# 0xk0ry/HTR-VT

Hardware: AMD Instinct MI355X
Metric: line-images/sec (64x1024, global B=128, 128 per GPU) fwd+bwd+CTC (higher is better)
Workload: dtype bf16; 1 GPU; HTR-VT (d768/4L/6h, nb_cls 80) training step: fwd + fused CTC + bwd + AdamW; image=1x64x1024, batch_per_gpu=128, global_batch=128, mask=span 0.4/8 (run/iam.sh), parallelism=dp1, graph_replay=False

## Files before the change

htr-vt_amd/_lib.py:

```python
from __future__ import annotations

import ctypes as C
import os

import torch

_HERE = os.path.dirname(os.path.abspath(__file__))
LIB_PATH = os.environ.get("HTRVT_LIB") or os.path.join(_HERE, "lib", "libhtrvt_hip.so")

F32, BF16 = 0, 1
KMAJOR, MNMAJOR = 0, 1
GATHER_NONE, GATHER_CONV_FWD, GATHER_CONV_DGRAD, GATHER_CONV_WGRAD = 0, 1, 2, 3

vp, i32, i64, f32, f64 = C.c_void_p, C.c_int32, C.c_int64, C.c_float, C.c_double


class RelayoutJob(C.Structure):
    _fields_ = [
        ("src", vp), ("dst0", vp), ("dst1", vp), ("kind", i32), ("d0", i32), ("d1", i32),
        ("taps", i32), ("cpad_in", i32), ("cpad_out", i32), ("row_taps", i32), ("tap0", i32),
        ("tile0", i32), ("tiles_x", i32), ("reserved_", i32 * 2),
    ]


# ... 6 lines not shown
        ("dtype", i32), ("a_layout", i32), ("b_layout", i32), ("gather", i32),
        ("M", i32), ("N", i32), ("K", i32),
        ("lda", i64), ("ldb", i64), ("ldc", i64),
        ("batch", i32), ("batch_inner", i32),
        ("sA_o", i64), ("sA_i", i64), ("sB_o", i64), ("sB_i", i64), ("sC_o", i64), ("sC_i", i64),
        ("split_k", i32), ("splitk_ws", vp),
        ("nB", i32), ("Hi", i32), ("Wi", i32), ("Ci", i32), ("Ho", i32), ("Wo", i32), ("Co", i32),
        ("kh", i32), ("kw", i32), ("sh", i32), ("sw", i32), ("ph", i32), ("pw", i32), ("Cpad", i32),
        ("cls_h", i32), ("cls_w", i32),
        ("A2", vp),
        ("alpha", f32), ("act", i32), ("c_f32", i32), ("accumulate", i32), ("tile", i32),
        ("bias", vp), ("colscale", vp), ("preact", vp), ("residual", vp), ("colstats", vp),
        ("relu_src", vp), ("bnb_x", vp * 2), ("bnb_mean", vp * 2), ("bnb_rstd", vp * 2), ("bnb_partial", vp * 2),
        ("bnb_tile0", i32), ("relu_scale", vp), ("relu_shift", vp), ("relu_bits", i32),
        ("A", vp), ("B", vp), ("C", vp),
    ]


PROTOTYPES = {
    "htrvt_version": (i32, []),
    "htrvt_last_error": (C.c_char_p, []),
    "htrvt_last_kernel": (C.c_char_p, []),
    "htrvt_gemm": (i32, [C.POINTER(GemmDesc), vp]),
    "htrvt_gemm_num_mtiles": (i32, [C.POINTER(GemmDesc)]),
    "htrvt_gemm_wgrad_tiling": (i32, [C.POINTER(GemmDesc), C.POINTER(i32), C.POINTER(i32)]),
    "htrvt_gemm_dgrad_merged_tiles": (i32, [C.POINTER(GemmDesc)]),
    "htrvt_img_stats": (i32, [vp, vp, i32, i32, f32, i32, vp]),
    "htrvt_conv1_fwd": (i32, [vp, vp, vp, vp, vp, i32, i32, i32, i32, i32, i32, vp]),
    "htrvt_stem_stats_rows": (i32, [i32, i32]),
    "htrvt_stem_stats": (i32, [vp, vp, vp, vp, vp, i32, i32, i32, i32, i32, vp]),
# ... 8 lines not shown
    "htrvt_softmax_rows": (i32, [vp, vp, i64, i32, i32, vp, i64, vp]),
    "htrvt_attn_supported": (i32, [i32, i32, i32]),
    "htrvt_attn_fwd": (i32, [vp, vp, vp, vp, i32, i32, i32, i32, f32, i32, vp]),
    "htrvt_attn_bwd": (i32, [vp, vp, vp, vp, vp, vp, vp, vp, i32, i32, i32, i32, f32, i32, vp]),
    "htrvt_seq_whiten_fwd": (i32, [vp, vp, vp, i32, i32, f32, i32, vp]),
    "htrvt_seq_whiten_bwd": (i32, [vp, vp, vp, vp, i32, i32, i32, i32, i32, vp]),
    "htrvt_layernorm_bwd_blocks": (i32, [i64]),
    "htrvt_layernorm_bwd": (i32, [vp, vp, vp, vp, vp, vp, vp, vp, i64, i32, i32, vp]),
    "htrvt_softmax_bwd_rows": (i32, [vp, vp, vp, i64, i32, f32, i32, vp]),
    "htrvt_colsum_workspace_floats": (C.c_size_t, [i64, i32]),
    "htrvt_colsum": (i32, [vp, i64, i32, i64, vp, vp, i32, i32, vp, vp]),
    "htrvt_rowsum_f32": (i32, [vp, i32, i32, vp, vp]),
    "htrvt_bn_bwd_blocks": (i32, [i64]),
    "htrvt_bn_bwd_reduce": (i32, [vp, vp, vp, vp, vp, vp, i64, i32, i32, vp]),
    "htrvt_bn_bwd_finalize": (i32, [vp, i32, i32, f32, vp, vp, vp, vp, vp, vp, vp]),
    "htrvt_bn_bwd_apply": (i32, [vp, vp, vp, vp, vp, vp, i64, i32, i32, vp]),
    "htrvt_bn_bwd_apply2": (i32, [vp, vp, vp, vp, vp, vp, vp, i64, i32, i32, vp]),
    "htrvt_maxpool_bwd": (i32, [vp, vp, vp, vp, vp, vp, i32, i32, i32, i32, i32, vp]),
    "htrvt_pool_tokens_bwd": (i32, [vp, vp, vp, vp, i32, i32, i32, i32, i32, vp]),
    "htrvt_conv1_bwd_rows": (i32, [i32, i32]),
    "htrvt_conv1_bwd_row_floats": (i32, [i32]),
    "htrvt_conv1_bwd": (i32, [vp] * 12 + [i32, i32, i32, i32, i32, i32, vp]),
    "htrvt_conv1_wgrad_blocks": (i32, [i32, i32]),
    "htrvt_conv1_wgrad": (i32, [vp, vp, vp, vp, vp, i32, i32, i32, i32, i32, i32, vp]),
    "htrvt_pack_conv_weight": (i32, [vp, vp, vp, i32, i32, i32, i32, i32, i32, vp]),
    "htrvt_pack_conv_weight_slots": (i32, [vp, vp, vp, i32, i32, i32, i32, i32, i32, i32, i32, vp]),
    "htrvt_unpack_conv_wgrad": (i32, [vp, vp, i32, i32, i32, i32, vp]),
    "htrvt_cast_f32": (i32, [vp, vp, i64, i32, vp]),
    "htrvt_relayout_plan": (i32, [vp, i32]),
    "htrvt_relayout": (i32, [vp, i32, i32, i32, vp]),
# ... 78 lines not shown
```

htr-vt_amd/csrc/bwd.hip:

```cpp
#include "common.h"

using namespace htrvt;

namespace {

constexpr int NT = 256;
constexpr int MAXC = 4;

inline int grid_for(long long work_items, int cap = 256 * 8) {
  long long g = (work_items + NT - 1) / NT;
  if (g > cap) g = cap;
  if (g < 1) g = 1;
  return (int)g;
}

template <typename T>
__global__ __launch_bounds__(NT) void seq_whiten_bwd_kernel(const float* __restrict__ dy, const float* __restrict__ y,
                                                            const float* __restrict__ stats, T* __restrict__ dx, int NC,
                                                            int C, int ldo) {
  __shared__ float red[8];
  const float* dys = dy + (long long)blockIdx.x * NC;
  const float* ys = y + (long long)blockIdx.x * NC;
  float s1 = 0.f, s2 = 0.f;
  for (int i = threadIdx.x; i < NC; i += NT) {
// ... 798 lines not shown
  dim3 grid(htrvt_bn_bwd_blocks(npix));
  DISPATCH_T(dtype, hipLaunchKernelGGL(bn_bwd_reduce_kernel<T>, grid, dim3(NT), smem, (hipStream_t)stream, (const T*)dy,
                                       (const T*)yact, (const T*)x, mean, rstd, partial, (long long)npix, C, nthr));
  return check_launch("bn_bwd_reduce");
}

extern "C" int htrvt_bn_bwd_finalize(const float* partial, int rows, int C, float count, const float* gamma,
                                     const float* mean, const float* rstd, float* dgamma, float* dbeta, float* coef,
                                     void* stream) {
  HTRVT_REQUIRE(partial && gamma && mean && rstd && dgamma && dbeta && coef, "htrvt_bn_bwd_finalize: null argument");
  hipLaunchKernelGGL(bn_bwd_finalize_kernel, dim3((C + 63) / 64), dim3(64), 0, (hipStream_t)stream, partial, rows, C, count,
                     gamma, mean, rstd, dgamma, dbeta, coef);
  return check_launch("bn_bwd_finalize");
}

extern "C" int htrvt_bn_bwd_apply(const void* dy, const void* yact, const void* x, const float* coef, void* dx, void* gout,
                                  int64_t npix, int C, int dtype, void* stream) {
  const int ch = dtype == HTRVT_BF16 ? 8 : 4;
  HTRVT_REQUIRE(C % ch == 0, "htrvt_bn_bwd_apply: C=%d unsupported", C);
  const long long nvec = npix * (C / ch);
  dim3 grid(grid_for(nvec));
  if (nvec * 16 >= BN_STREAM_BYTES) {
    DISPATCH_T(dtype, hipLaunchKernelGGL((bn_bwd_apply_kernel<T, true>), grid, dim3(NT), (size_t)3 * C * sizeof(float), (hipStream_t)stream, (const T*)dy,
                                         (const T*)yact, (const T*)x, coef, (T*)dx, (T*)gout, nvec, C));
  } else {
    DISPATCH_T(dtype, hipLaunchKernelGGL((bn_bwd_apply_kernel<T, false>), grid, dim3(NT), (size_t)3 * C * sizeof(float), (hipStream_t)stream, (const T*)dy,
                                         (const T*)yact, (const T*)x, coef, (T*)dx, (T*)gout, nvec, C));
  }
  return check_launch("bn_bwd_apply");
}
// ... 111 lines not shown
```

htr-vt_amd/csrc/gemm.hip:

```cpp
#include "gemm_common.h"

using namespace htrvt;

namespace {

constexpr int NTHREADS = 256;

template <typename T, int ROWS, int LAYOUT>
struct TileGeom {
  static constexpr int SZ = ET<T>::SZ;
  static constexpr int BK = ET<T>::BK;
  static constexpr int STRIDE = (LAYOUT == HTRVT_KMAJOR) ? 128 : (ROWS * SZ + 64);
  static constexpr int LROWS = (LAYOUT == HTRVT_KMAJOR) ? ROWS : BK;
  static constexpr int BYTES = STRIDE * LROWS;
  static constexpr int NLOAD = ROWS / 32;
  static constexpr int CPR = (LAYOUT == HTRVT_KMAJOR) ? 8 : (ROWS * SZ / 16);
};

template <typename T, int ROWS, int LAYOUT, int ROLE>
struct Loader {
  using G = TileGeom<T, ROWS, LAYOUT>;
  static constexpr int SZ = G::SZ, CH = ET<T>::CH, NL = G::NLOAD;
  uint4 reg[NL];
  const char* ptr[NL];
// ... 246 lines not shown
            for (int j = 0; j < TN; ++j)
              acc[i][j] = __builtin_amdgcn_mfma_f32_32x32x2f32((&fa[i].x)[jj], (&fb[j].x)[jj], acc[i][j], 0, 0, 0);
      }
    }
    if (more) {
      la.commit(nxt);
      lb.commit(nxt + GA::BYTES);
    }
    __syncthreads();
  }

  gemm_epilogue<T, TM, TN, 2, BN, NTHREADS>(acc, p, Cb, coff, m0 + wm * TM * 32, n0 + wn * TN * 32, wm, n0, tile_m, lane, smem);
}

__global__ __launch_bounds__(NTHREADS) void splitk_reduce_kernel(const float* __restrict__ ws, float* __restrict__ C, int M, int N,
                                                                 long long ldc, int nsl, int accumulate) {
  const long long mn = (long long)M * N;
  const int n4 = N >> 2;
  for (long long i = (long long)blockIdx.x * NTHREADS + threadIdx.x; i < (long long)M * n4; i += (long long)gridDim.x * NTHREADS) {
    const int m = (int)(i / n4), c = (int)(i - (long long)m * n4);
    const float4* src = reinterpret_cast<const float4*>(ws + (long long)m * N) + c;
    float4 a = *src;
    int z = 1;
    for (; z + 8 <= nsl; z += 8) {
      float4 b[8];
#pragma unroll
      for (int u = 0; u < 8; ++u) b[u] = *reinterpret_cast<const float4*>(reinterpret_cast<const float*>(src) + (z + u) * mn);
#pragma unroll
      for (int u = 0; u < 8; ++u) {
        a.x += b[u].x; a.y += b[u].y; a.z += b[u].z; a.w += b[u].w;
      }
// ... 203 lines not shown
      HTRVT_REQUIRE(diff > 0 && diff + (long long)d->nB * d->Ho * d->Wo * d->Co * 2 < (1ll << 31) - 64,
                    "htrvt_gemm: A2 must lie behind A, both inside 2 GiB");
      p.tapsel[p.ntapsel++] = (unsigned char)(d->kh * d->kw);
      p.extra_off = (unsigned)diff;
    }
    HTRVT_REQUIRE(d->M == d->nB * p.Hq * p.Wq && d->K == p.ntapsel * d->Cpad && d->N == d->Ci,
                  "htrvt_gemm: parity-class dgrad extents inconsistent (expected M=%d K=%d)", d->nB * p.Hq * p.Wq,
                  p.ntapsel * d->Cpad);
  }
  p.tappack = 0;
  for (int t = 0; t < 12; ++t) p.tappack |= (unsigned long long)(p.tapsel[t] & 15) << (4 * t);
  const int zdim = p.split_k > 1 ? p.split_k : (d->batch > 1 ? d->batch : 1);
  HTRVT_REQUIRE((long long)p.tiles_m * p.tiles_n < (1ll << 31) && zdim < 65536, "htrvt_gemm: grid too large");
  hipStream_t st = (hipStream_t)stream;
  p.slab_stride = 0;
  if (p.split_k > 1 && d->splitk_ws != nullptr) {
    p.C = reinterpret_cast<char*>(d->splitk_ws);
    p.ldc = d->N;
    p.accumulate = 0;
    p.slab_stride = (long long)d->M * d->N;
    const int rc = launch_main(d, p, bm, bn, zdim, st);
    if (rc) return rc;
    long long items = (long long)d->M * (d->N / 4);
    int grid = (int)((items + NTHREADS - 1) / NTHREADS);
    if (grid > 2048) grid = 2048;
    hipLaunchKernelGGL(splitk_reduce_kernel, dim3(grid), dim3(NTHREADS), 0, st, d->splitk_ws, reinterpret_cast<float*>(d->C), d->M,
                       d->N, (long long)d->ldc, p.split_k, d->accumulate);
    return check_launch("splitk_reduce");
  }
  return launch_main(d, p, bm, bn, zdim, st);
}

static int launch_main(const HtrvtGemmDesc* d, KParams& p, int bm, int bn, int zdim, hipStream_t st) {
  const bool cls = d->gather == HTRVT_GATHER_CONV_DGRAD && d->cls_h >= 0;
  const bool fused_bwd = d->relu_src != nullptr || d->bnb_partial[0] != nullptr;
  if (d->dtype == HTRVT_BF16 && d->tile != 1) {
    KParams q = p;
    int r = gemm8p_try_launch(d, q, zdim, st);
    if (r != 0) return r < 0 ? r : 0;
    q = p;
    r = gemm8pt_try_launch(d, q, zdim, st);
    if (r != 0) return r < 0 ? r : 0;
// ... 21 lines not shown
```

htr-vt_amd/csrc/gemm8p.hip:

```cpp
#include <stdlib.h>

#include "gemm_common.h"

using namespace htrvt;

namespace htrvt {
int gemm8p_dispatch_plain(int bn, int epi, const KParams&, int, hipStream_t);
int gemm8pp_dispatch_plain(int bn, int epi, const KParams&, int nwg, hipStream_t);
int gemm8pt_dispatch(const KParams&, int zdim, hipStream_t);
int gemm8p_dispatch_conv(int bn, int gather, int epi, const KParams&, int, hipStream_t);
}

namespace {

int ilog2_exact(int v) {
  if (v <= 0 || (v & (v - 1))) return -1;
  int s = 0;
  while ((1 << s) < v) ++s;
  return s;
}

bool extents_ok(const HtrvtGemmDesc* d) {
  const long long lim = (1ll << 31) - 64;
  long long a, b = (long long)d->N * d->ldb * 2;
// ... 48 lines not shown
}

bool gemm8pt_serves(const HtrvtGemmDesc* d) {
  if (d->tile != 0 && d->tile != 16) return false;
  if (d->dtype != HTRVT_BF16 || d->gather != HTRVT_GATHER_NONE || d->a_layout != HTRVT_MNMAJOR || d->b_layout != HTRVT_MNMAJOR) return false;
  if (!d->c_f32 || d->batch > 1 || d->M < 256 || d->N < 256 || d->K < 256) return false;
  if (d->tile == 0 && (long long)((d->M + 255) / 256) * ((d->N + 255) / 256) < 16) return false;
  if ((d->M & 7) || (d->N & 7) || (d->lda & 7) || (d->ldb & 7) || (d->ldc & 3)) return false;
  if ((reinterpret_cast<unsigned long long>(d->A) & 15) || (reinterpret_cast<unsigned long long>(d->B) & 15) || (reinterpret_cast<unsigned long long>(d->C) & 15)) return false;
  if (d->bias != nullptr || d->act != 0 || d->preact != nullptr || d->residual != nullptr || d->colstats != nullptr || d->colscale != nullptr) return false;
  const long long lim = (1ll << 31) - 64;
  if ((long long)d->K * d->lda * 2 >= lim || (long long)d->K * d->ldb * 2 >= lim) return false;
  return true;
}

int gemm8pt_try_launch(const HtrvtGemmDesc* d, KParams& p, int zdim, hipStream_t st) {
  if (!gemm8pt_serves(d)) return 0;
  if (p.split_k > 1 ? p.slab_stride == 0 : p.accumulate != 0) return 0;
  p.tiles_m = (d->M + 255) / 256;
  p.tiles_n = (d->N + 255) / 256;
  return gemm8pt_dispatch(p, zdim, st);
}

int gemm8p_try_launch(const HtrvtGemmDesc* d, KParams& p, int zdim, hipStream_t st) {
  if (!gemm8p_serves(d)) return 0;
  const int bn = gemm8p_pick_bn(d);
  int epi = 0;
  if (d->residual != nullptr) epi |= E_RES;
  if (d->act == 1) epi |= E_GELU;
  if (d->act == 2) epi |= E_GELUGRAD;
// ... 42 lines not shown
```

htr-vt_amd/csrc/gemm8p_impl.h:

```cpp
#pragma once
#include <type_traits>

#include "gemm_common.h"

using namespace htrvt;

namespace g8 {

constexpr int BK = 64;

typedef int i32x2_t __attribute__((ext_vector_type(2)));
typedef float f32x4_t __attribute__((ext_vector_type(4)));
using I0 = std::integral_constant<int, 0>;
using I1 = std::integral_constant<int, 1>;

template <int BN_, int WARPS_M_, int WARPS_N_>
struct Cfg {
  static constexpr int BM = 256, BN = BN_, WARPS_M = WARPS_M_, WARPS_N = WARPS_N_;
  static_assert(WARPS_M * WARPS_N == 8, "8 waves");
  static constexpr int HM = BM / 2, HN = BN / 2;
  static constexpr int SM = HM / WARPS_M, SN = HN / WARPS_N;
  static constexpr int MT = SM / 16, NT = SN / 16;
  static_assert(SM % 16 == 0 && SN % 16 == 0 && (NT == 2 || NT == 3), "quadrant shape");
  static constexpr int A_HALF = HM * 128, B_HALF = HN * 128;
// ... 259 lines not shown
  if ((wave >> 2) == 1) __builtin_amdgcn_s_barrier();
}

template <class F>
__device__ __forceinline__ void mfma_phase(F&& mma) {
  __builtin_amdgcn_s_barrier();
  asm volatile("s_waitcnt lgkmcnt(0)" ::: "memory");
  __builtin_amdgcn_sched_barrier(0);
  __builtin_amdgcn_s_setprio(1);
  mma();
  __builtin_amdgcn_s_setprio(0);
  __builtin_amdgcn_sched_barrier(0);
  __builtin_amdgcn_s_barrier();
}

template <int BUFI, int LGKM1, class RA, class RB, class SA, class SB, class MMA>
__device__ __forceinline__ void ktile8p(RA& readA, RB& readB, SA& stageA, SB& stageB, MMA& mma) {
  using BX = std::integral_constant<int, BUFI>;
  using BY = std::integral_constant<int, BUFI ^ 1>;
  readB(I0{}, BX{});
  __builtin_amdgcn_sched_barrier(0);
  readA(I0{}, BX{});
  __builtin_amdgcn_sched_barrier(0);
  stageA(I1{}, BY{});
  asm volatile("s_waitcnt lgkmcnt(%0)" ::"n"(LGKM1) : "memory");
  mfma_phase([&] { mma(I0{}, I0{}); });
  readB(I1{}, BX{});
  __builtin_amdgcn_sched_barrier(0);
  stageB(I0{}, BX{});
  mfma_phase([&] { mma(I0{}, I1{}); });
  readA(I1{}, BX{});
  __builtin_amdgcn_sched_barrier(0);
  stageA(I0{}, BX{});
  mfma_phase([&] { mma(I1{}, I1{}); });
  stageB(I1{}, BX{});
  asm volatile("s_waitcnt vmcnt(6)" ::: "memory");
  mfma_phase([&] { mma(I1{}, I0{}); });
}

__device__ __forceinline__ void drain8p(int wave) {
  if ((wave >> 2) == 0) __builtin_amdgcn_s_barrier();
  asm volatile("s_waitcnt vmcnt(0)" ::: "memory");
}

template <class C, int GATHER, int EPI, class P>
__device__ __forceinline__ void gemm8p_body(const P& p, const int block_x) {
  constexpr int MT = C::MT, NT = C::NT;
  extern __shared__ __attribute__((aligned(16))) char smem[];

  const int id = xcd_tile_id(block_x, p.tiles_m * p.tiles_n);
// ... 340 lines not shown
```

htr-vt_amd/csrc/gemm8pt_impl.h:

```cpp
#pragma once
#include "gemm8p_impl.h"

namespace g8 {

__device__ __forceinline__ int tswz(int k) { return ((k & 3) | (((k >> 3) & 1) << 2)) << 1; }

struct TLoad {
  unsigned off[2][2];
  int klocal[2];
  unsigned kstep;
  int k0;
  i32x4_t rsrc;

  __device__ __forceinline__ void init(const char* base, long long ld, int mn0, int dim, int kbeg, int wave, int lane) {
    rsrc = make_rsrc(base);
    k0 = kbeg;
    kstep = (unsigned)(BK * ld * 2);
#pragma unroll
    for (int i = 0; i < 2; ++i) {
      const int pi = wave + 8 * i;
      const int kl = 4 * pi + (lane >> 4);
      klocal[i] = kl;
      const int cs = (lane & 15) ^ tswz(kl);
#pragma unroll
// ... 8 lines not shown
#pragma unroll
    for (int i = 0; i < 2; ++i) {
      const unsigned voff = (k0 + klocal[i] < kend) ? off[H][i] : OOB;
      dma16(rsrc, __builtin_amdgcn_readfirstlane(lds_half + (wave + 8 * i) * 1024), voff);
    }
    if constexpr (H == 1) {
      k0 += BK;
#pragma unroll
      for (int i = 0; i < 2; ++i)
#pragma unroll
        for (int h = 0; h < 2; ++h) off[h][i] = off[h][i] < OOB ? off[h][i] + kstep : OOB;
    }
  }
};

template <class P>
__device__ __forceinline__ void gemm8pt_body(const P& p, const int block_x) {
  using C = Cfg<256, 2, 4>;
  constexpr int MT = C::MT, NT = C::NT;
  extern __shared__ __attribute__((aligned(16))) char smem[];

  const int id = xcd_tile_id(block_x, p.tiles_m * p.tiles_n);
  const int tile_m = id / p.tiles_n, tile_n = id - tile_m * p.tiles_n;
  const int m0 = tile_m * C::BM, n0 = tile_n * C::BN;
  const int z = blockIdx.z;
  const int kbeg = z * p.kchunk;
  const int kend = (kbeg + p.kchunk < p.K) ? kbeg + p.kchunk : p.K;

  const int lane = threadIdx.x & 63;
  const int wave = __builtin_amdgcn_readfirstlane(threadIdx.x >> 6);
  const int wr = wave / C::WARPS_N, wc = wave - wr * C::WARPS_N;
// ... 53 lines not shown
  };
  auto readB = [&](auto yc, auto bufc) {
    constexpr int Y = decltype(yc)::value;
    const char* half = smem + decltype(bufc)::value * C::BUF + (Y ? OB1 : OB0);
#pragma unroll
    for (int j = 0; j < NT; ++j) {
      fb[Y][j][0] = ldtr(half, rdB[j]);
      fb[Y][j][1] = ldtr(half, rdB[j] + 32 * 256);
    }
  };
  auto mma = [&](auto xc, auto yc) {
    constexpr int X = decltype(xc)::value, Y = decltype(yc)::value;
    mma_quadrant<false>(acc[X][Y], fb[Y], fa);
  };
  constexpr int LGKM1 = 15;
  prologue8p(stageA, stageB, wave);
  int kt = 0;
  for (; kt + 1 < nkt; kt += 2) {
    ktile8p<0, LGKM1>(readA, readB, stageA, stageB, mma);
    ktile8p<1, LGKM1>(readA, readB, stageA, stageB, mma);
  }
  if (kt < nkt) ktile8p<0, LGKM1>(readA, readB, stageA, stageB, mma);
  drain8p(wave);

  const int g = lane >> 4, jr = lane & 15;
  float* Cf = reinterpret_cast<float*>(p.C) + (p.slab_stride > 0 ? (long long)z * p.slab_stride : 0ll);
  const float alpha = p.alpha;
#pragma unroll
  for (int x = 0; x < 2; ++x)
#pragma unroll
    for (int i = 0; i < MT; ++i) {
      const int m = m0 + x * C::HM + wr * C::SM + 16 * i + jr;
      if (m < p.M) {
        float* row = Cf + (long long)m * p.ldc;
#pragma unroll
        for (int y = 0; y < 2; ++y)
#pragma unroll
          for (int j = 0; j < NT; ++j) {
            const int n = n0 + y * C::HN + wc * C::SN + 16 * j + 4 * g;
            if (n < p.N) *reinterpret_cast<f32x4_t*>(row + n) = acc[x][y][i][j] * alpha;
          }
      }
    }
}

__global__ __launch_bounds__(512) void gemm8pt_kernel(const KParams p) {
  typedef const __attribute__((address_space(4))) KParams KP;
  (void)p;
  KP* kp = (KP*)__builtin_amdgcn_kernarg_segment_ptr();
  gemm8pt_body(*kp, (int)blockIdx.x);
}

inline int launch_t(const KParams& p, int zdim, hipStream_t st) {
  using C = Cfg<256, 2, 4>;
  if (int rc = allow_dynamic_lds<gemm8pt_kernel>(C::LDS_BYTES, "gemm8pt_kernel")) return rc;
  hipLaunchKernelGGL(gemm8pt_kernel, dim3(p.tiles_m * p.tiles_n, 1, zdim), dim3(512), C::LDS_BYTES, st, p);
  set_last_kernel("gemm8pt_kernel");
  const int rc = check_launch("gemm8pt_kernel");
  return rc ? rc : 1;
}

}
```

htr-vt_amd/csrc/gemm_common.h:

```cpp
#pragma once
#include "common.h"

namespace htrvt {

typedef __attribute__((ext_vector_type(8))) __bf16 bf16x8_t;
typedef __attribute__((ext_vector_type(4))) short s16x4_t;
typedef __attribute__((ext_vector_type(8))) short s16x8_t;
typedef __attribute__((ext_vector_type(16))) float f32x16_t;
typedef int i32x4_t __attribute__((ext_vector_type(4)));

constexpr unsigned OOB = 0x80000000u;

__device__ __forceinline__ void dma16(const i32x4_t& rsrc, unsigned lds_addr, unsigned voff) {
  unsigned keep;
  asm volatile(
      "s_nop 4\n\t"
      "s_mov_b32 %0, m0\n\t"
      "s_mov_b32 m0, %2\n\t"
      "s_nop 0\n\t"
      "buffer_load_dwordx4 %1, %3, 0 offen lds\n\t"
      "s_mov_b32 m0, %0"
      : "=&s"(keep)
      : "v"(voff), "s"(lds_addr), "s"(rsrc)
      : "memory");
// ... 51 lines not shown
  int wo_shift, howo_shift;
  int cls_h, cls_w, Hq, Wq, ntapsel;
  int wq_shift, hwq_shift;
  unsigned char tapsel[12];
  unsigned long long tappack;
  unsigned extra_off;
  const char* relu_src;
  int relu_bits;
  const char* bnb_x[2];
  const float* bnb_mean[2];
  const float* bnb_rstd[2];
  float* bnb_partial[2];
  int bnb_tile0;
  const float* relu_sc;
  const float* relu_sf;
};

inline bool gemm_small_m_prefers_bn128(const HtrvtGemmDesc* d) {
  if (d->tile != 0 || d->gather != HTRVT_GATHER_NONE || d->dtype != HTRVT_BF16) return false;
  if (d->a_layout != HTRVT_KMAJOR || d->b_layout != HTRVT_KMAJOR || d->batch > 1 || d->split_k > 1) return false;
  if (d->N > 1024 || d->N % 128 != 0) return false;
  const long long tiles192 = (long long)((d->M + 255) / 256) * ((d->N + 191) / 192);
  return tiles192 <= 128;
}

__device__ __forceinline__ float gelu_erf(float x) { return 0.5f * x * (1.0f + erff(x * 0.70710678118654752440f)); }
__device__ __forceinline__ float gelu_erf_grad(float x) {
  return 0.5f * (1.0f + erff(x * 0.70710678118654752440f)) + x * 0.39894228040143267794f * __expf(-0.5f * x * x);
}

// ... 129 lines not shown
          q += red[(w * BN + c) * 2 + 1];
        }
        float* dst = p.colstats + (long long)tile_m * 2 * p.N;
        dst[n] = a;
        dst[p.N + n] = q;
      }
    }
  }
}

int gemm_dma_try_launch(const HtrvtGemmDesc* d, KParams& p, int zdim, hipStream_t st);
int gemm_dma_num_mtiles(const HtrvtGemmDesc* d);
int gemm8p_try_launch(const HtrvtGemmDesc* d, KParams& p, int zdim, hipStream_t st);
int gemm8pt_try_launch(const HtrvtGemmDesc* d, KParams& p, int zdim, hipStream_t st);
bool gemm8pt_serves(const HtrvtGemmDesc* d);

}
```

htr-vt_amd/csrc/gemm_hwgrad.hip:

```cpp
#include "gemm_hwgrad_impl.h"

namespace htrvt {

int gemm_hwgrad_bn(const HtrvtGemmDesc* d);
bool gemm_hwgrad_is16(const HtrvtGemmDesc* d) {
  if (gemm_hwgrad_bn(d) != 192) return false;
  if (d->sw == 2) return d->Cpad % 96 == 0 && d->tile == 13;
  return d->Cpad % 128 != 0 && d->Cpad % 96 == 0 && (d->tile == 0 || d->tile == 13);
}
int gemm_hwgrad_cc(const HtrvtGemmDesc* d) { return gemm_hwgrad_is16(d) ? 96 : ((d->Cpad % 128 == 0 || d->tile != 17) ? 128 : 64); }
bool gemm_hwgrad_pair(const HtrvtGemmDesc* d) { return !gemm_hwgrad_is16(d) && d->Cpad % 128 != 0 && d->tile != 17; }
int gemm_hwgrad_bn(const HtrvtGemmDesc* d) {
  const int p192 = (d->N + 191) / 192 * 192, p128 = (d->N + 127) / 128 * 128;
  return p192 <= p128 ? 192 : 128;
}

bool gemm_hwgrad_serves(const HtrvtGemmDesc* d) {
  if (d->gather != HTRVT_GATHER_CONV_WGRAD || d->dtype != HTRVT_BF16) return false;
  if (d->tile != 0 && d->tile != 13 && d->tile != 17 && d->tile != 18) return false;
  if (d->kh != 3 || d->kw != 3 || (d->sh != 1 && d->sh != 2) || (d->sw != 1 && d->sw != 2) || d->ph != 1 || d->pw != 1) return false;
  if (d->Ho != (d->Hi - 1) / d->sh + 1 || (d->Wo % 64) != 0) return false;
  if (d->sw == 1 ? d->Wo != d->Wi : ((d->Wi & 1) || d->Wo != d->Wi / 2 || !gemm_hwgrad_is16(d))) return false;
  if (!d->c_f32 || d->batch > 1 || d->Cpad % 64 != 0 || d->M != 9 * d->Cpad || d->N != d->Co) return false;
  if (d->bias != nullptr || d->act != 0 || d->preact != nullptr || d->residual != nullptr || d->colstats != nullptr) return false;
// ... 19 lines not shown
    p.tiles_m = (3 * (d->Cpad / 64) + 1) / 2;
    return bn == 192 ? launch_hwgrad<128, 192, true>(p, zdim, st) : launch_hwgrad<128, 128, true>(p, zdim, st);
  }
  p.tiles_m = 3 * (d->Cpad / cc);
  if (cc == 128 && bn == 192) return launch_hwgrad<128, 192>(p, zdim, st);
  if (cc == 128 && bn == 128) return launch_hwgrad<128, 128>(p, zdim, st);
  if (cc == 64 && bn == 192) return launch_hwgrad<64, 192>(p, zdim, st);
  return launch_hwgrad<64, 128>(p, zdim, st);
}

}

extern "C" int htrvt_gemm_wgrad_tiling(const HtrvtGemmDesc* d, int* tile_rows, int* tile_cols) {
  if (d == nullptr) return 0;
  if (d->gather == HTRVT_GATHER_NONE) {
    if (!htrvt::gemm8pt_serves(d) || !(d->split_k > 1 ? d->accumulate != 0 : d->accumulate == 0)) return 0;
    if (tile_rows) *tile_rows = 256;
    if (tile_cols) *tile_cols = 256;
    return ((d->M + 255) / 256) * ((d->N + 255) / 256);
  }
  if (!htrvt::gemm_hwgrad_serves(d)) return 0;
  if (tile_rows) *tile_rows = 3 * htrvt::gemm_hwgrad_cc(d);
  if (tile_cols) *tile_cols = htrvt::gemm_hwgrad_bn(d);
  return htrvt::gemm_hwgrad_tiles(d);
}
```

htr-vt_amd/engine.py:

```python
from __future__ import annotations

import torch

from . import ops, seq_ops
from ._lib import lib, check, RelayoutJob, RELAYOUT_PACK_CONV, RELAYOUT_CAST_TRANSPOSE, RELAYOUT_UNPACK_WGRAD, RELAYOUT_ARG_JOBS
from .ops import KMAJOR, MNMAJOR, GATHER_CONV_DGRAD, GATHER_CONV_FWD, GATHER_CONV_WGRAD, ConvGeom, cpad, dt, gemm, ptr, stream

LN_EPS = 1e-6
WHITEN_EPS = 1e-5
BN_EPS = 1e-5
BN_MOMENTUM = 0.1


def _pool_len(n, k, s, p):
    return (n + 2 * p - k) // s + 1


def stem_tokens(H, W):
    h, w = _pool_len(H, 3, 2, 1), W
    h, w = _pool_len(h, 3, 2, 1), _pool_len(w, 3, 1, 1)
    h, w = _pool_len(h, 3, 2, 1), w
    h, w = _pool_len(h, 3, 2, 1), _pool_len(w, 3, 2, 1)
    h, w = _pool_len(h, 3, 2, 1), _pool_len(w, 3, 2, 1)
    h, w = _pool_len(h, 3, 2, 1), _pool_len(w, 3, 1, 1)
# ... 356 lines not shown
        cands = [1, 2, 3, 4, 5, 6, 7] + list(range(8, smax, 8)) + ([10, 12, 14, 20, 28] if tiling is not None else [])
        if conv or tiling is not None:
            cands = sorted(set(cands) | set(range(8, 65)))
        for s in cands:
            if Kred // s < 512:
                continue
            blocks = tiles * s
            rounds = (blocks + 255) // 256
            t = flops / 1.0e15 * (rounds * 256.0 / blocks) + blocks * bm * bn * 4 / (2.5e12 if self.deterministic and s > 1 else 1.3e12)
            if s > 1 and s % 8:
                t *= 1.02
            if best_t is None or t < best_t:
                best, best_t = s, t
        return best

    def _splitk_ws(self, sk, Mo, No):
        if sk > 1 and self.deterministic and No % 4:
            if not getattr(self, "_warned_atomics", False):
                import warnings
                warnings.warn(f"htrvt_amd: split-K weight gradient with {No} output columns (not a multiple of 4) uses float "
                              "atomics: results are not bitwise reproducible although Engine.deterministic is set")
                self._warned_atomics = True
            return None
        if sk <= 1 or not self.deterministic:
            return None
        return self._empty(sk, Mo, No, dtype=torch.float32)

    def _on_side(self, fn, *tensors):
        if not self._side_active:
            return fn()
        if self._side is None:
            self._side = torch.cuda.Stream(device=self.dev)
        self._side.wait_stream(torch.cuda.current_stream())
        for t in tensors:
            t.record_stream(self._side)
        with torch.cuda.stream(self._side):
            return fn()

    def _wgrad_stream(self):
        return self._side if (self._side is not None and self._side_active) else None

# ... 26 lines not shown
            d.A, d.B, d.C = dyp, ptr(x), ptr(dw)
            tr_, tc_ = ctypes.c_int32(0), ctypes.c_int32(0)
            nt = lib.htrvt_gemm_wgrad_tiling(ctypes.byref(d), ctypes.byref(tr_), ctypes.byref(tc_))
            if nt > 0:
                tiling = (nt, tr_.value, tc_.value)
        sk = self._split_k(N, K, M, tiling=tiling)
        if self.split and not plain:
            dy3, _, _ = self._split_act(dy, N, cat=True, planes=False)
            _, xh, xl = self._split_act(x, K, cat=False, planes=True)
            for a_off, b_ in ((0, xh), (0, xl), (N, xh)):
                gemm(dy3, b_, dw, dtype=self.gdt, M=N, N=K, K=M, lda=3 * N, ldb=K, ldc=K, a_layout=MNMAJOR, b_layout=MNMAJOR,
                     split_k=sk, accumulate=True, c_f32=True, splitk_ws=self._splitk_ws(sk, N, K), a_off=a_off)
            if dbias is not None:
                ops.colsum(dy, M, N, N, dbias, dti=self.dti)
            return
        gemm(dy, x, dw, dtype=self.dtype, M=N, N=K, K=M, lda=ld, ldb=K, ldc=K, a_layout=MNMAJOR, b_layout=MNMAJOR,
             split_k=sk, accumulate=True, c_f32=True, splitk_ws=self._splitk_ws(sk, N, K), a_off=off)
        if dbias is not None:
            ops.colsum(dyp, M, N, ld, dbias, dti=self.dti)

    def conv_fwd(self, x, wf, g: ConvGeom, want_stats, bn=None, relu=False, residual=None):
        M = g.B * g.Ho * g.Wo
        cpi = cpad(g.Ci, self.dtype)
        y = self._empty(g.B, g.Ho, g.Wo, g.Co)
        cs, rows = None, 0
        if want_stats:
            rows = ops.gemm_num_mtiles(M, g.Co, self.gdt, gather=GATHER_CONV_FWD)
            cs = self._empty(rows + 64, 2, g.Co, dtype=torch.float32)
        kw = {}
        if bn is not None:
            kw = dict(colscale=bn[0], bias=bn[1], residual=residual, act=3 if relu else 0)
        if self.split:
            x3, _, _ = self._split_act(x, g.Ci)
# ... 238 lines not shown
        return y

    def bn_backward(self, dy, yact, x, prefix, P, G, mean, rstd, want_g=False, out=None):
        C = x.shape[-1]
        npix = x.numel() // C
        nblk = lib.htrvt_bn_bwd_blocks(npix)
        partial = self._empty(nblk, 2, C, dtype=torch.float32)
        check(lib.htrvt_bn_bwd_reduce(ptr(dy), ptr(yact), ptr(x), ptr(mean), ptr(rstd), ptr(partial), npix, C, self.dti,
                                      stream()), "bn_bwd_reduce")
        return self.bn_backward_finish(partial, nblk, dy, yact, x, prefix, P, G, mean, rstd, want_g, out=out)

    def bn_backward_coef(self, partial, rows, x, prefix, P, G, mean, rstd):
        C = x.shape[-1]
        npix = x.numel() // C
        coef = self._empty(3, C, dtype=torch.float32)
        src = partial
        if rows > 64:
            red = self._zeros(2 * C)
            ops.colsum(partial, rows, 2 * C, 2 * C, red, dti=0)
            src, rows = red, 1
        count = float(npix) if self._bn_train else -1.0
        check(lib.htrvt_bn_bwd_finalize(ptr(src), rows, C, count, ptr(P[prefix + ".weight"]), ptr(mean), ptr(rstd),
                                        ptr(G[prefix + ".weight"]), ptr(G[prefix + ".bias"]), ptr(coef), stream()),
              "bn_bwd_finalize")
        return coef

    def bn_backward_finish(self, partial, rows, g, yact, x, prefix, P, G, mean, rstd, want_g=False, out=None):
        C = x.shape[-1]
        npix = x.numel() // C
        coef = self.bn_backward_coef(partial, rows, x, prefix, P, G, mean, rstd)
        dx = torch.empty_like(x) if out is None else out
        gout = torch.empty_like(x) if want_g else None
        check(lib.htrvt_bn_bwd_apply(ptr(g), ptr(yact), ptr(x), ptr(coef), ptr(dx), ptr(gout), npix, C, self.dti, stream()),
              "bn_bwd_apply")
        return dx, gout

    def ln_fwd(self, x, gamma, beta, save):
        return seq_ops.layernorm_fwd(x, gamma, beta, self.s.ln_eps, save)

# ... 548 lines not shown
```

htr-vt_amd/ops.py:

```python
from __future__ import annotations

import ctypes as C

import torch

from . import _lib
from ._lib import BF16, F32, GATHER_CONV_DGRAD, GATHER_CONV_FWD, GATHER_CONV_WGRAD, KMAJOR, MNMAJOR, GemmDesc, check, lib

_ENV_TILE = 0


def dt(dtype: torch.dtype) -> int:
    if dtype == torch.float32:
        return F32
    if dtype == torch.bfloat16:
        return BF16
    raise TypeError(f"unsupported dtype {dtype}")


def bk_of(dtype: torch.dtype) -> int:
    return 64 if dtype == torch.bfloat16 else 32


def cpad(c: int, dtype: torch.dtype) -> int:
# ... 20 lines not shown
        self.sh, self.sw = stride
        self.ph = self.pw = pad
        self.Ho = (Hi + 2 * pad - k) // self.sh + 1
        self.Wo = (Wi + 2 * pad - k) // self.sw + 1
        self.taps = k * k

    def fill(self, d: GemmDesc):
        d.nB, d.Hi, d.Wi, d.Ci, d.Ho, d.Wo, d.Co = self.B, self.Hi, self.Wi, self.Ci, self.Ho, self.Wo, self.Co
        d.kh, d.kw, d.sh, d.sw, d.ph, d.pw = self.kh, self.kw, self.sh, self.sw, self.ph, self.pw


def gemm(A, B, Cout, *, dtype, M, N, K, lda, ldb, ldc, a_layout=KMAJOR, b_layout=KMAJOR, gather=0, geom=None,
         Cpad=0, batch=1, batch_inner=1, sA=(0, 0), sB=(0, 0), sC=(0, 0), split_k=1, alpha=1.0, act=0, c_f32=False,
         accumulate=False, bias=None, colscale=None, preact=None, residual=None, colstats=None, tile=0,
         a_off=0, b_off=0, c_off=0, cls=None, relu_src=None, bnb=None, bnb_tile0=0, splitk_ws=None, a2=None, relu_bn=None,
         relu_bits=False):
    d = GemmDesc()
    d.dtype = dt(dtype)
    d.a_layout, d.b_layout, d.gather = a_layout, b_layout, gather
    d.M, d.N, d.K = M, N, K
    d.lda, d.ldb, d.ldc = lda, ldb, ldc
    d.batch, d.batch_inner = batch, batch_inner
    d.sA_o, d.sA_i = sA
    d.sB_o, d.sB_i = sB
    d.sC_o, d.sC_i = sC
    d.split_k = split_k
    d.splitk_ws = ptr(splitk_ws)
    d.cls_h, d.cls_w = (-1, -1) if cls is None else cls
    d.A2 = ptr(a2)
    if geom is not None:
        geom.fill(d)
        d.Cpad = Cpad
    d.alpha = alpha
    d.act = act
    d.c_f32 = 1 if c_f32 else 0
    d.accumulate = 1 if accumulate else 0
    d.tile = tile or _ENV_TILE
    d.bias = ptr(bias)
    d.colscale = ptr(colscale)
    d.preact = ptr(preact)
    d.residual = ptr(residual)
    d.colstats = ptr(colstats)
# ... 56 lines not shown
```

include/htrvt.h:

```cpp
#ifndef HTRVT_H
#define HTRVT_H

#include <stddef.h>
#include <stdint.h>

#ifdef __cplusplus
extern "C" {
#endif

#define HTRVT_F32 0
#define HTRVT_BF16 1

#define HTRVT_KMAJOR 0
#define HTRVT_MNMAJOR 1

#define HTRVT_GATHER_NONE 0
#define HTRVT_GATHER_CONV_FWD 1
#define HTRVT_GATHER_CONV_DGRAD 2
#define HTRVT_GATHER_CONV_WGRAD 3

int htrvt_version(void);
const char* htrvt_last_error(void);
const char* htrvt_last_kernel(void);

// ... 20 lines not shown
  void* preact;
  const void* residual;
  float* colstats;
  const void* relu_src;
  const void* bnb_x[2];
  const float* bnb_mean[2];
  const float* bnb_rstd[2];
  float* bnb_partial[2];
  int32_t bnb_tile0;
  const float* relu_scale;
  const float* relu_shift;
  int32_t relu_bits;
  const void* A;
  const void* B;
  void* C;
} HtrvtGemmDesc;

int htrvt_gemm(const HtrvtGemmDesc* d, void* stream);
int htrvt_gemm_num_mtiles(const HtrvtGemmDesc* d);
int htrvt_gemm_wgrad_tiling(const HtrvtGemmDesc* d, int* tile_rows, int* tile_cols);
int htrvt_gemm_dgrad_merged_tiles(const HtrvtGemmDesc* d);

int htrvt_img_stats(const void* img, float* stats, int B, int HW, float eps, int img_u8, void* stream);
int htrvt_conv1_fwd(const void* img, const float* stats, const float* w, void* out, float* colstats,
                    int B, int H, int W, int C, int dtype, int img_u8, void* stream);
int htrvt_stem_stats_rows(int B, int H);
int htrvt_stem_stats(const void* img, const float* stats, const float* w, float* partial, float* colstats, int B, int H,
                     int W, int C, int img_u8, void* stream);
int htrvt_stem_fwd(const void* img, const float* stats, const float* w, const float* scale, const float* shift, void* y,
                   uint8_t* idx, int B, int H, int W, int C, int dtype, int img_u8, void* stream);
// ... 31 lines not shown
                         int dtype, void* stream);
int htrvt_layernorm_bwd_blocks(int64_t rows);
int htrvt_layernorm_bwd(const void* dy, const void* x, const float* mean, const float* rstd, const float* gamma,
                        const void* dres, void* dx, float* partial, int64_t rows, int D, int dtype, void* stream);
int htrvt_softmax_bwd_rows(const void* p, const float* dp, void* ds, int64_t rows, int n, float scale, int dtype,
                           void* stream);
size_t htrvt_colsum_workspace_floats(int64_t rows, int cols);
int htrvt_colsum(const void* x, int64_t rows, int cols, int64_t ld, float* out, const float* keep, int keep_mod,
                 int dtype, float* workspace, void* stream);
int htrvt_rowsum_f32(const float* partial, int rows, int cols, float* out, void* stream);
int htrvt_bn_bwd_blocks(int64_t npix);
int htrvt_bn_bwd_reduce(const void* dy, const void* yact, const void* x, const float* mean, const float* rstd,
                        float* partial, int64_t npix, int C, int dtype, void* stream);
int htrvt_bn_bwd_finalize(const float* partial, int rows, int C, float count, const float* gamma, const float* mean,
                          const float* rstd, float* dgamma, float* dbeta, float* coef , void* stream);
int htrvt_bn_bwd_apply(const void* dy, const void* yact, const void* x, const float* coef, void* dx, void* gout,
                       int64_t npix, int C, int dtype, void* stream);
int htrvt_bn_bwd_apply2(const void* g, const void* x1, const float* coef1, void* dx1, const void* x2, const float* coef2,
                        void* dx2, int64_t npix, int C, int dtype, void* stream);
int htrvt_maxpool_bwd(const void* dpool, const uint8_t* idx, const void* x, const float* scale, const float* shift,
                      void* g, int B, int H, int W, int C, int dtype, void* stream);
int htrvt_pool_tokens_bwd(const void* dtok, const void* x, const float* keep, void* dx, int B, int H, int N, int D,
                          int dtype, void* stream);
int htrvt_conv1_wgrad_blocks(int B, int H);
int htrvt_conv1_wgrad(const void* img, const float* stats, const void* dy, float* dw, float* partial,
                      int B, int H, int W, int C, int dtype, int img_u8, void* stream);

int htrvt_conv1_bwd_rows(int B, int H);
int htrvt_conv1_bwd_row_floats(int C);
int htrvt_conv1_bwd(const void* img, const float* stats, const void* dpool, const uint8_t* idx, const float* w,
// ... 139 lines not shown
```

Baseline: 4118 line-images/s.

## Fuse bias-gradient row sums into wgrad GEMM and merge BN bwd reduce/finalize

Adds a rowsum variant of the 8-phase MN-major wgrad GEMM kernel that accumulates dbias from the A fragments it already loads, using bf16 dot2 against ones. This replaces the separate colsum pass over dy. Split-k slabs write per-slice row sums that the split-k reduce kernel folds in. A second change adds a C entry point that chains a multi-split column reduction with the BN backward finalize. It drops the zero-fill and a Python-level launch, and the reduction now uses several splits instead of one. Risks are extra register pressure and extra VALU work in the GEMM main loop for the waves that compute the sums, plus the N<=1536 restriction on the fused path.

```diff
diff --git a/htr-vt_amd/_lib.py b/htr-vt_amd/_lib.py
--- a/htr-vt_amd/_lib.py
+++ b/htr-vt_amd/_lib.py
@@ -44,6 +44,7 @@
         ("relu_src", vp), ("bnb_x", vp * 2), ("bnb_mean", vp * 2), ("bnb_rstd", vp * 2), ("bnb_partial", vp * 2),
         ("bnb_tile0", i32), ("relu_scale", vp), ("relu_shift", vp), ("relu_bits", i32),
         ("A", vp), ("B", vp), ("C", vp),
+        ("rowsum", vp),
     ]
 
 
@@ -82,6 +83,7 @@
     "htrvt_bn_bwd_blocks": (i32, [i64]),
     "htrvt_bn_bwd_reduce": (i32, [vp, vp, vp, vp, vp, vp, i64, i32, i32, vp]),
     "htrvt_bn_bwd_finalize": (i32, [vp, i32, i32, f32, vp, vp, vp, vp, vp, vp, vp]),
+    "htrvt_bn_bwd_coef": (i32, [vp, i32, i32, f32, vp, vp, vp, vp, vp, vp, vp, vp]),
     "htrvt_bn_bwd_apply": (i32, [vp, vp, vp, vp, vp, vp, i64, i32, i32, vp]),
     "htrvt_bn_bwd_apply2": (i32, [vp, vp, vp, vp, vp, vp, vp, i64, i32, i32, vp]),
     "htrvt_maxpool_bwd": (i32, [vp, vp, vp, vp, vp, vp, i32, i32, i32, i32, i32, vp]),
diff --git a/htr-vt_amd/csrc/bwd.hip b/htr-vt_amd/csrc/bwd.hip
--- a/htr-vt_amd/csrc/bwd.hip
+++ b/htr-vt_amd/csrc/bwd.hip
@@ -836,6 +836,25 @@
   return check_launch("bn_bwd_finalize");
 }
 
+extern "C" int htrvt_bn_bwd_coef(const float* partial, int rows, int C, float count, const float* gamma, const float* mean,
+                                 const float* rstd, float* dgamma, float* dbeta, float* coef, float* workspace, void* stream) {
+  HTRVT_REQUIRE(partial && gamma && mean && rstd && dgamma && dbeta && coef, "htrvt_bn_bwd_coef: null argument");
+  HTRVT_REQUIRE(rows > 0 && C > 0, "htrvt_bn_bwd_coef: rows=%d C=%d", rows, C);
+  if (rows > 64) {
+    HTRVT_REQUIRE(workspace != nullptr && C % 2 == 0, "htrvt_bn_bwd_coef: %d rows need a workspace of 64*2*C floats and an even C", rows);
+    int splits = colsum_splits(rows);
+    if (splits < 2) splits = 2;
+    const int cols = 2 * C;
+    hipLaunchKernelGGL(colsum_kernel<float>, dim3((cols / 4 + 31) / 32, (unsigned)splits), dim3(1024), 0, (hipStream_t)stream, partial,
+                       (long long)rows, cols, (long long)cols, (float*)nullptr, (const float*)nullptr, 1, workspace);
+    partial = workspace;
+    rows = splits;
+  }
+  hipLaunchKernelGGL(bn_bwd_finalize_kernel, dim3((C + 63) / 64), dim3(64), 0, (hipStream_t)stream, partial, rows, C, count,
+                     gamma, mean, rstd, dgamma, dbeta, coef);
+  return check_launch("bn_bwd_coef");
+}
+
 extern "C" int htrvt_bn_bwd_apply(const void* dy, const void* yact, const void* x, const float* coef, void* dx, void* gout,
                                   int64_t npix, int C, int dtype, void* stream) {
   const int ch = dtype == HTRVT_BF16 ? 8 : 4;
diff --git a/htr-vt_amd/csrc/gemm.hip b/htr-vt_amd/csrc/gemm.hip
--- a/htr-vt_amd/csrc/gemm.hip
+++ b/htr-vt_amd/csrc/gemm.hip
@@ -284,7 +284,15 @@
 }
 
 __global__ __launch_bounds__(NTHREADS) void splitk_reduce_kernel(const float* __restrict__ ws, float* __restrict__ C, int M, int N,
-                                                                 long long ldc, int nsl, int accumulate) {
+                                                                 long long ldc, int nsl, int accumulate,
+                                                                 const float* __restrict__ rs_ws, float* __restrict__ rowsum) {
+  if (rowsum != nullptr) {
+    for (int m = blockIdx.x * NTHREADS + threadIdx.x; m < M; m += gridDim.x * NTHREADS) {
+      float a = rs_ws[m];
+      for (int z = 1; z < nsl; ++z) a += rs_ws[(long long)z * M + m];
+      rowsum[m] += a;
+    }
+  }
   const long long mn = (long long)M * N;
   const int n4 = N >> 2;
   for (long long i = (long long)blockIdx.x * NTHREADS + threadIdx.x; i < (long long)M * n4; i += (long long)gridDim.x * NTHREADS) {
@@ -518,18 +526,22 @@
   HTRVT_REQUIRE((long long)p.tiles_m * p.tiles_n < (1ll << 31) && zdim < 65536, "htrvt_gemm: grid too large");
   hipStream_t st = (hipStream_t)stream;
   p.slab_stride = 0;
+  HTRVT_REQUIRE(d->rowsum == nullptr || (d->dtype == HTRVT_BF16 && d->tile != 1 && gemm8pt_serves_launch(d)),
+                "htrvt_gemm: rowsum needs a launch the MN-major 8-phase kernel serves (ask htrvt_gemm_wgrad_tiling first)");
+  p.rowsum = d->rowsum;
   if (p.split_k > 1 && d->splitk_ws != nullptr) {
     p.C = reinterpret_cast<char*>(d->splitk_ws);
     p.ldc = d->N;
     p.accumulate = 0;
     p.slab_stride = (long long)d->M * d->N;
+    if (d->rowsum != nullptr) p.rowsum = d->splitk_ws + p.split_k * p.slab_stride;
     const int rc = launch_main(d, p, bm, bn, zdim, st);
     if (rc) return rc;
     long long items = (long long)d->M * (d->N / 4);
     int grid = (int)((items + NTHREADS - 1) / NTHREADS);
     if (grid > 2048) grid = 2048;
     hipLaunchKernelGGL(splitk_reduce_kernel, dim3(grid), dim3(NTHREADS), 0, st, d->splitk_ws, reinterpret_cast<float*>(d->C), d->M,
-                       d->N, (long long)d->ldc, p.split_k, d->accumulate);
+                       d->N, (long long)d->ldc, p.split_k, d->accumulate, p.rowsum, d->rowsum);
     return check_launch("splitk_reduce");
   }
   return launch_main(d, p, bm, bn, zdim, st);
diff --git a/htr-vt_amd/csrc/gemm8p.hip b/htr-vt_amd/csrc/gemm8p.hip
--- a/htr-vt_amd/csrc/gemm8p.hip
+++ b/htr-vt_amd/csrc/gemm8p.hip
@@ -86,6 +86,14 @@
   return true;
 }
 
+bool gemm8pt_serves_launch(const HtrvtGemmDesc* d) {
+  if (!gemm8pt_serves(d)) return false;
+  if (d->split_k > 1 ? d->accumulate == 0 : d->accumulate != 0) return false;
+  if (d->rowsum != nullptr && d->split_k > 1 && d->splitk_ws == nullptr) return false;
+  if (d->rowsum != nullptr && d->N > 1536) return false;
+  return true;
+}
+
 int gemm8pt_try_launch(const HtrvtGemmDesc* d, KParams& p, int zdim, hipStream_t st) {
   if (!gemm8pt_serves(d)) return 0;
   if (p.split_k > 1 ? p.slab_stride == 0 : p.accumulate != 0) return 0;
diff --git a/htr-vt_amd/csrc/gemm8p_impl.h b/htr-vt_amd/csrc/gemm8p_impl.h
--- a/htr-vt_amd/csrc/gemm8p_impl.h
+++ b/htr-vt_amd/csrc/gemm8p_impl.h
@@ -297,8 +297,13 @@
   __builtin_amdgcn_s_barrier();
 }
 
-template <int BUFI, int LGKM1, class RA, class RB, class SA, class SB, class MMA>
-__device__ __forceinline__ void ktile8p(RA& readA, RB& readB, SA& stageA, SB& stageB, MMA& mma) {
+struct NoAux {
+  template <class X>
+  __device__ __forceinline__ void operator()(X) const {}
+};
+
+template <int BUFI, int LGKM1, class RA, class RB, class SA, class SB, class MMA, class AUX = NoAux>
+__device__ __forceinline__ void ktile8p(RA& readA, RB& readB, SA& stageA, SB& stageB, MMA& mma, AUX aux = AUX{}) {
   using BX = std::integral_constant<int, BUFI>;
   using BY = std::integral_constant<int, BUFI ^ 1>;
   readB(I0{}, BX{});
@@ -311,12 +316,14 @@
   readB(I1{}, BX{});
   __builtin_amdgcn_sched_barrier(0);
   stageB(I0{}, BX{});
+  aux(I0{});
   mfma_phase([&] { mma(I0{}, I1{}); });
   readA(I1{}, BX{});
   __builtin_amdgcn_sched_barrier(0);
   stageA(I0{}, BX{});
   mfma_phase([&] { mma(I1{}, I1{}); });
   stageB(I1{}, BX{});
+  aux(I1{});
   asm volatile("s_waitcnt vmcnt(6)" ::: "memory");
   mfma_phase([&] { mma(I1{}, I0{}); });
 }
diff --git a/htr-vt_amd/csrc/gemm8pt_impl.h b/htr-vt_amd/csrc/gemm8pt_impl.h
--- a/htr-vt_amd/csrc/gemm8pt_impl.h
+++ b/htr-vt_amd/csrc/gemm8pt_impl.h
@@ -46,7 +46,18 @@
   }
 };
 
-template <class P>
+typedef __attribute__((ext_vector_type(2))) __bf16 bf16x2_t;
+
+__device__ __forceinline__ float frag_sum(float acc, const bf16x8_t& f) {
+  const bf16x2_t ones = __builtin_bit_cast(bf16x2_t, 0x3F803F80);
+  acc = __builtin_amdgcn_fdot2_f32_bf16(__builtin_shufflevector(f, f, 0, 1), ones, acc, false);
+  acc = __builtin_amdgcn_fdot2_f32_bf16(__builtin_shufflevector(f, f, 2, 3), ones, acc, false);
+  acc = __builtin_amdgcn_fdot2_f32_bf16(__builtin_shufflevector(f, f, 4, 5), ones, acc, false);
+  acc = __builtin_amdgcn_fdot2_f32_bf16(__builtin_shufflevector(f, f, 6, 7), ones, acc, false);
+  return acc;
+}
+
+template <bool ROWSUM, class P>
 __device__ __forceinline__ void gemm8pt_body(const P& p, const int block_x) {
   using C = Cfg<256, 2, 4>;
   constexpr int MT = C::MT, NT = C::NT;
@@ -130,16 +141,46 @@
     mma_quadrant<false>(acc[X][Y], fb[Y], fa);
   };
   constexpr int LGKM1 = 15;
+  const bool do_rs = ROWSUM && tile_n == 0 && wc == 0;
+  float rs[2][MT];
+#pragma unroll
+  for (int x = 0; x < 2; ++x)
+#pragma unroll
+    for (int i = 0; i < MT; ++i) rs[x][i] = 0.f;
+  auto aux = [&](auto xc) {
+    if constexpr (ROWSUM) {
+      constexpr int X = decltype(xc)::value;
+      if (do_rs) {
+#pragma unroll
+        for (int i = 0; i < MT; ++i) rs[X][i] = frag_sum(frag_sum(rs[X][i], fa[i][0]), fa[i][1]);
+      }
+    }
+  };
   prologue8p(stageA, stageB, wave);
   int kt = 0;
   for (; kt + 1 < nkt; kt += 2) {
-    ktile8p<0, LGKM1>(readA, readB, stageA, stageB, mma);
-    ktile8p<1, LGKM1>(readA, readB, stageA, stageB, mma);
-  }
-  if (kt < nkt) ktile8p<0, LGKM1>(readA, readB, stageA, stageB, mma);
+    ktile8p<0, LGKM1>(readA, readB, stageA, stageB, mma, aux);
+    ktile8p<1, LGKM1>(readA, readB, stageA, stageB, mma, aux);
+  }
+  if (kt < nkt) ktile8p<0, LGKM1>(readA, readB, stageA, stageB, mma, aux);
   drain8p(wave);
 
   const int g = lane >> 4, jr = lane & 15;
+  if constexpr (ROWSUM) {
+    if (do_rs) {
+      float* dst = p.rowsum + (p.slab_stride > 0 ? (long long)z * p.M : 0ll);
+#pragma unroll
+      for (int x = 0; x < 2; ++x)
+#pragma unroll
+        for (int i = 0; i < MT; ++i) {
+          float v = rs[x][i];
+          v += __shfl_xor(v, 16);
+          v += __shfl_xor(v, 32);
+          const int m = m0 + x * C::HM + wr * C::SM + 16 * i + jr;
+          if (g == 0 && m < p.M) dst[m] = p.slab_stride > 0 ? v : dst[m] + v;
+        }
+    }
+  }
   float* Cf = reinterpret_cast<float*>(p.C) + (p.slab_stride > 0 ? (long long)z * p.slab_stride : 0ll);
   const float alpha = p.alpha;
 #pragma unroll
@@ -164,11 +205,25 @@
   typedef const __attribute__((address_space(4))) KParams KP;
   (void)p;
   KP* kp = (KP*)__builtin_amdgcn_kernarg_segment_ptr();
-  gemm8pt_body(*kp, (int)blockIdx.x);
+  gemm8pt_body<false>(*kp, (int)blockIdx.x);
+}
+
+__global__ __launch_bounds__(512) void gemm8pt_rowsum_kernel(const KParams p) {
+  typedef const __attribute__((address_space(4))) KParams KP;
+  (void)p;
+  KP* kp = (KP*)__builtin_amdgcn_kernarg_segment_ptr();
+  gemm8pt_body<true>(*kp, (int)blockIdx.x);
 }
 
 inline int launch_t(const KParams& p, int zdim, hipStream_t st) {
   using C = Cfg<256, 2, 4>;
+  if (p.rowsum != nullptr) {
+    if (int rc = allow_dynamic_lds<gemm8pt_rowsum_kernel>(C::LDS_BYTES, "gemm8pt_rowsum_kernel")) return rc;
+    hipLaunchKernelGGL(gemm8pt_rowsum_kernel, dim3(p.tiles_m * p.tiles_n, 1, zdim), dim3(512), C::LDS_BYTES, st, p);
+    set_last_kernel("gemm8pt_rowsum_kernel");
+    const int rc = check_launch("gemm8pt_rowsum_kernel");
+    return rc ? rc : 1;
+  }
   if (int rc = allow_dynamic_lds<gemm8pt_kernel>(C::LDS_BYTES, "gemm8pt_kernel")) return rc;
   hipLaunchKernelGGL(gemm8pt_kernel, dim3(p.tiles_m * p.tiles_n, 1, zdim), dim3(512), C::LDS_BYTES, st, p);
   set_last_kernel("gemm8pt_kernel");
diff --git a/htr-vt_amd/csrc/gemm_common.h b/htr-vt_amd/csrc/gemm_common.h
--- a/htr-vt_amd/csrc/gemm_common.h
+++ b/htr-vt_amd/csrc/gemm_common.h
@@ -89,6 +89,7 @@
   int bnb_tile0;
   const float* relu_sc;
   const float* relu_sf;
+  float* rowsum;
 };
 
 inline bool gemm_small_m_prefers_bn128(const HtrvtGemmDesc* d) {
@@ -248,5 +249,6 @@
 int gemm8p_try_launch(const HtrvtGemmDesc* d, KParams& p, int zdim, hipStream_t st);
 int gemm8pt_try_launch(const HtrvtGemmDesc* d, KParams& p, int zdim, hipStream_t st);
 bool gemm8pt_serves(const HtrvtGemmDesc* d);
-
-}
+bool gemm8pt_serves_launch(const HtrvtGemmDesc* d);
+
+}
diff --git a/htr-vt_amd/csrc/gemm_hwgrad.hip b/htr-vt_amd/csrc/gemm_hwgrad.hip
--- a/htr-vt_amd/csrc/gemm_hwgrad.hip
+++ b/htr-vt_amd/csrc/gemm_hwgrad.hip
@@ -57,7 +57,7 @@
 extern "C" int htrvt_gemm_wgrad_tiling(const HtrvtGemmDesc* d, int* tile_rows, int* tile_cols) {
   if (d == nullptr) return 0;
   if (d->gather == HTRVT_GATHER_NONE) {
-    if (!htrvt::gemm8pt_serves(d) || !(d->split_k > 1 ? d->accumulate != 0 : d->accumulate == 0)) return 0;
+    if (!htrvt::gemm8pt_serves_launch(d)) return 0;
     if (tile_rows) *tile_rows = 256;
     if (tile_cols) *tile_cols = 256;
     return ((d->M + 255) / 256) * ((d->N + 255) / 256);
diff --git a/htr-vt_amd/engine.py b/htr-vt_amd/engine.py
--- a/htr-vt_amd/engine.py
+++ b/htr-vt_amd/engine.py
@@ -394,7 +394,7 @@
                 best, best_t = s, t
         return best
 
-    def _splitk_ws(self, sk, Mo, No):
+    def _splitk_ws(self, sk, Mo, No, rowsum=False):
         if sk > 1 and self.deterministic and No % 4:
             if not getattr(self, "_warned_atomics", False):
                 import warnings
@@ -404,7 +404,7 @@
             return None
         if sk <= 1 or not self.deterministic:
             return None
-        return self._empty(sk, Mo, No, dtype=torch.float32)
+        return self._empty(sk * (Mo * No + (Mo if rowsum else 0)), dtype=torch.float32)
 
     def _on_side(self, fn, *tensors):
         if not self._side_active:
@@ -461,9 +461,16 @@
             if dbias is not None:
                 ops.colsum(dy, M, N, N, dbias, dti=self.dti)
             return
+        want_rs = dbias is not None and tiling is not None
+        ws = self._splitk_ws(sk, N, K, rowsum=want_rs)
+        rs = None
+        if want_rs:
+            d.split_k, d.splitk_ws, d.rowsum = sk, ptr(ws), ptr(dbias)
+            if lib.htrvt_gemm_wgrad_tiling(ctypes.byref(d), None, None) > 0:
+                rs = dbias
         gemm(dy, x, dw, dtype=self.dtype, M=N, N=K, K=M, lda=ld, ldb=K, ldc=K, a_layout=MNMAJOR, b_layout=MNMAJOR,
-             split_k=sk, accumulate=True, c_f32=True, splitk_ws=self._splitk_ws(sk, N, K), a_off=off)
-        if dbias is not None:
+             split_k=sk, accumulate=True, c_f32=True, splitk_ws=ws, a_off=off, rowsum=rs)
+        if dbias is not None and rs is None:
             ops.colsum(dyp, M, N, ld, dbias, dti=self.dti)
 
     def conv_fwd(self, x, wf, g: ConvGeom, want_stats, bn=None, relu=False, residual=None):
@@ -732,15 +739,11 @@
         C = x.shape[-1]
         npix = x.numel() // C
         coef = self._empty(3, C, dtype=torch.float32)
-        src = partial
-        if rows > 64:
-            red = self._zeros(2 * C)
-            ops.colsum(partial, rows, 2 * C, 2 * C, red, dti=0)
-            src, rows = red, 1
+        ws = self._empty(64, 2 * C, dtype=torch.float32) if rows > 64 else None
         count = float(npix) if self._bn_train else -1.0
-        check(lib.htrvt_bn_bwd_finalize(ptr(src), rows, C, count, ptr(P[prefix + ".weight"]), ptr(mean), ptr(rstd),
-                                        ptr(G[prefix + ".weight"]), ptr(G[prefix + ".bias"]), ptr(coef), stream()),
-              "bn_bwd_finalize")
+        check(lib.htrvt_bn_bwd_coef(ptr(partial), rows, C, count, ptr(P[prefix + ".weight"]), ptr(mean), ptr(rstd),
+                                    ptr(G[prefix + ".weight"]), ptr(G[prefix + ".bias"]), ptr(coef), ptr(ws), stream()),
+              "bn_bwd_coef")
         return coef
 
     def bn_backward_finish(self, partial, rows, g, yact, x, prefix, P, G, mean, rstd, want_g=False, out=None):
diff --git a/htr-vt_amd/ops.py b/htr-vt_amd/ops.py
--- a/htr-vt_amd/ops.py
+++ b/htr-vt_amd/ops.py
@@ -58,7 +58,7 @@
          Cpad=0, batch=1, batch_inner=1, sA=(0, 0), sB=(0, 0), sC=(0, 0), split_k=1, alpha=1.0, act=0, c_f32=False,
          accumulate=False, bias=None, colscale=None, preact=None, residual=None, colstats=None, tile=0,
          a_off=0, b_off=0, c_off=0, cls=None, relu_src=None, bnb=None, bnb_tile0=0, splitk_ws=None, a2=None, relu_bn=None,
-         relu_bits=False):
+         relu_bits=False, rowsum=None):
     d = GemmDesc()
     d.dtype = dt(dtype)
     d.a_layout, d.b_layout, d.gather = a_layout, b_layout, gather
@@ -70,6 +70,7 @@
     d.sC_o, d.sC_i = sC
     d.split_k = split_k
     d.splitk_ws = ptr(splitk_ws)
+    d.rowsum = ptr(rowsum)
     d.cls_h, d.cls_w = (-1, -1) if cls is None else cls
     d.A2 = ptr(a2)
     if geom is not None:
diff --git a/include/htrvt.h b/include/htrvt.h
--- a/include/htrvt.h
+++ b/include/htrvt.h
@@ -58,6 +58,7 @@
   const void* A;
   const void* B;
   void* C;
+  float* rowsum;
 } HtrvtGemmDesc;
 
 int htrvt_gemm(const HtrvtGemmDesc* d, void* stream);
@@ -119,6 +120,8 @@
                         float* partial, int64_t npix, int C, int dtype, void* stream);
 int htrvt_bn_bwd_finalize(const float* partial, int rows, int C, float count, const float* gamma, const float* mean,
                           const float* rstd, float* dgamma, float* dbeta, float* coef , void* stream);
+int htrvt_bn_bwd_coef(const float* partial, int rows, int C, float count, const float* gamma, const float* mean,
+                      const float* rstd, float* dgamma, float* dbeta, float* coef , float* workspace, void* stream);
 int htrvt_bn_bwd_apply(const void* dy, const void* yact, const void* x, const float* coef, void* dx, void* gout,
                        int64_t npix, int C, int dtype, void* stream);
 int htrvt_bn_bwd_apply2(const void* g, const void* x1, const float* coef1, void* dx1, const void* x2, const float* coef2,
```

Result: no change. 4133 line-images/s (median of 6 runs) (+0.4%).
